# Audio-WestlakeU/FN-SSL

Measured on AMD Instinct MI355X. Metric: TF-frames/sec DP-IPD forward, 4-mic 257-bin x 300-frame, higher is better.
Workload: dtype f32; 1 GPU; BASELINE configs[1]: FN-SSL (online) DP-IPD forward, waveform->STFT->features->3x(full-band BiLSTM + narrow-band LSTM)->head; 32 utterances/GPU x 4 mics ('MM' = 6 pairs) x 257 bins x 300 frames, fp32; frame = one STFT frame of one utterance; stream_chunk_frames=0, utterances_per_gpu=32, global_batch=32, mics=4, pairs_per_utterance=6, frames=300, bins=257, parallelism=dp1 (utterance shards, no collective), chunk_pairs=0

## Files before the change

### fn-ssl_amd/csrc/lstm_f32c.h

```cpp
#pragma once

#include "lstm_static.h"

namespace fnssl_lstm {

constexpr int kF32cWaves = 16;

struct F32ClusterParams {
  unsigned* tags;
  unsigned* status;
  int clusters_per_dir;
  int groups_per_cluster;
  unsigned spin_limit;
  int stall_member;
  int rotate;
  int prio_mode;
};

template <int HH, int NV0, int NS0, int MODE, bool ABLRT = false, int DRIFT = 2, int NW_ = kF32cWaves, int GS = 1>
__global__ void __launch_bounds__(NW_ * 64) lstm_f32c_kernel(const LstmParams p, const F32ClusterParams cp) {
  constexpr int H = HH, NS = H / 16, NW = NW_;
  constexpr int NWS = NW / GS;
  static_assert((GS == 1 || GS == 4) && NW % GS == 0 && (NWS & (NWS - 1)) == 0, "gate split: whole slots, a power of two of them");
  constexpr bool SUM = (MODE & kSum) != 0, SAVE = (MODE & kSave) != 0;
  constexpr bool CAT = (MODE & kHas2) != 0;
  constexpr int QPS = 1 + NV0 + NS0 + NS;
  constexpr int XD = NW_ > 12 ? 4 : 8;
  constexpr bool STRH = H == 256 && GS == 1 && NW_ > 8;
  static_assert((CAT ? NS0 == 1 : !(NV0 && NS0)) && (NV0 == 0 || NV0 % XD == 0) && (H == 128 || H == 256),
                "blocks of src0, or its remainder alone, or blocks of src0 + the remainder quad of src2");
  static_assert(H == 128 || NW_ <= 8 || STRH, "H = 256 with the row of h_{t-1} held: at most two waves per SIMD (register budget)");
  static_assert(!STRH || (NV0 >= XD && (NV0 + NS) % XD == 0), "streamed row: the ring depth divides the block count");
  static_assert(GS == 1 || (!SAVE && !ABLRT), "gate split: inference kernels only");
  extern __shared__ __attribute__((aligned(16))) char smem[];
  const int ABL = ABLRT ? p.ablate : 0;

  const int b = blockIdx.x;
  const int m = (b >> 3) % NS;
  const int cl = ((b >> 3) / NS) * 8 + (b & 7);
  if (cl >= cp.clusters_per_dir * p.ndir) return;
  const int dir = cl / cp.clusters_per_dir;
  const int ck = cl - dir * cp.clusters_per_dir;
  const int g0 = ck * cp.groups_per_cluster;
  const int g1 = g0 + cp.groups_per_cluster < p.ntasks ? g0 + cp.groups_per_cluster : p.ntasks;
  if (__hip_atomic_load(cp.status, __ATOMIC_RELAXED, __HIP_MEMORY_SCOPE_AGENT) != 0) return;
  if (cl == 0 && m == cp.stall_member) return;

  const int lane = threadIdx.x & 63;
  const int n = lane & 15, g = lane >> 4;
  const int w = __builtin_amdgcn_readfirstlane((int)(threadIdx.x >> 6));
  const int ws = GS == 1 ? w : (w >> 2);
  const int gate = GS == 1 ? 0 : (w & 3);
  const bool rev = dir == 1;
  const unsigned vlane = lane * 16;

  {
    const v4f* src = reinterpret_cast<const v4f*>(reinterpret_cast<const char*>(p.wpack[dir]) + (size_t)(m * QPS) * 4096);
    v4f* dst = reinterpret_cast<v4f*>(smem);
    for (int i = threadIdx.x; i < QPS * 4 * 64; i += NW * 64) dst[i] = src[i];
  }
  char* const xch = smem + QPS * 4096;
  unsigned* const xcnt = reinterpret_cast<unsigned*>(xch + NWS * 2 * 4 * 1024);
  if (GS > 1 && threadIdx.x < NWS) xcnt[threadIdx.x] = 0;
  __syncthreads();
  const char* const lds_rd = smem + lane * 16;
  auto rec = [&](int q, int j) { return *reinterpret_cast<const v4f*>(lds_rd + (q * 4 + j) * 1024); };
  auto rec1 = [&](int q, int j) { return *reinterpret_cast<const float*>(lds_rd + (q * 4 + j) * 1024 + 4 * gate); };

  const unsigned st0 = (unsigned)(p.src0.st * 4), sto = (unsigned)(p.out_st * 4), stk = SUM ? (unsigned)(p.skip.st * 4) : 0u;
  const unsigned st2 = CAT ? (unsigned)(p.src2.st * 4) : 0u;
  const unsigned cy = (unsigned)p.carry;
  unsigned* const tag_cl = cp.tags + (size_t)cl * cp.groups_per_cluster * NS;
  const v4f zero4 = v4f{0.f, 0.f, 0.f, 0.f};

  unsigned pub_val = 0;
  unsigned* pub_tag = nullptr;
  auto pub_flush = [&]() {
    if (pub_tag) {
      asm volatile("s_waitcnt vmcnt(0)" ::: "memory");
      if (lane == 0) __hip_atomic_store(pub_tag, pub_val, __ATOMIC_RELAXED, __HIP_MEMORY_SCOPE_AGENT);
      pub_tag = nullptr;
    }
  };

  struct Grp {
    unsigned vo0, voo, vok, voo2, vo2 = 0;
    bool valid;
    int task, step;
  };
  auto locate = [&](int task, int qo0, int qi0, Grp& gr, rsrc_t& rx0, rsrc_t& ro, rsrc_t& rsk, rsrc_t& ro2, rsrc_t& rx2) {
    const int q0 = task * 16;
    gr.valid = q0 + n < p.nseq;
    const int d = q0 + n < p.nseq ? n : p.nseq - 1 - q0;
    const bool crossed = qi0 + d >= p.q_inner;
    auto one = [&](const float* base, long long so, long long si, int extra, unsigned& voff) {
      const long long delta = (long long)d * si + (crossed ? so - (long long)p.q_inner * si : 0ll);
      voff = (unsigned)(delta * 4) + (unsigned)(extra * 4);
      return make_rsrc(base + ((long long)qo0 * so + (long long)qi0 * si));
    };
    rx0 = one(p.src0.p, p.src0.so, p.src0.si, (NS0 && !CAT) ? g : 4 * g, gr.vo0);
    if constexpr (CAT) rx2 = one(p.src2.p, p.src2.so, p.src2.si, g, gr.vo2);
    ro = one(p.out, p.out_so, p.out_si, dir * H + 4 * g, gr.voo);
    gr.vok = gr.voo2 = 0;
    rsk = SUM ? one(p.skip.p, p.skip.so, p.skip.si, dir * H + 4 * g, gr.vok) : rx0;
    ro2 = SUM ? one(p.out_sum, p.out_so, p.out_si, dir * H + 4 * g, gr.voo2) : ro;
  };
  auto tt_of = [&](int step) { return (unsigned)(rev ? p.nsteps - 1 - step : step); };
  auto rc_of = [&](int task) {
    return make_rsrc(cell_record<NS>(p.cscratch, p.ntasks, dir, task));
  };

  if (g0 + ws >= g1) return;
  unsigned long long clk0 = 0, rt0 = 0;
  if (ABLRT && (ABL & 512)) {
    clk0 = __builtin_amdgcn_s_memtime();
    rt0 = __builtin_amdgcn_s_memrealtime();
  }
  bool dead = false;
  auto bounded_wait = [&](auto ready, auto reload, int sleep, unsigned code) {
    for (unsigned spins = 0; !ready(); ++spins) {
      if (GS > 1) __builtin_amdgcn_s_sleep(1); else if (sleep == 8) __builtin_amdgcn_s_sleep(8); else __builtin_amdgcn_s_sleep(16);
      reload();
      const bool out = spins > cp.spin_limit;
      if (out || (spins & 63) == 63) {
        if (out) {
          if (lane == 0) __hip_atomic_store(cp.status, code | (unsigned)(cl & 0xffff), __ATOMIC_RELAXED, __HIP_MEMORY_SCOPE_AGENT);
          return false;
        }
        if (__hip_atomic_load(cp.status, __ATOMIC_RELAXED, __HIP_MEMORY_SCOPE_AGENT) != 0) return false;
      }
    }
    return true;
  };
  const int NGR = g1 - g0;
  const bool rot = cp.rotate && NGR >= 2 * NWS;
  const int FULL = rot ? (NGR / NWS) * NWS : NGR, LEFT = NGR - FULL;
  const bool single = GS == 1 && g0 + ws + NWS >= g1;
  Grp cur, nxt;
  rsrc_t rx0, ro, rsk, ro2, rx2, nrx0, nro, nrsk, nro2, nrx2;
  v4f xr[XD];
  float xs0 = 0.f;
  v4f cprev = zero4, skipv = zero4;
  unsigned tagv = 0, tagd = 0;
  auto request = [&](const Grp& gr, rsrc_t qx0, rsrc_t qsk, bool with_c, bool with_x = true) {
    const unsigned tt = tt_of(gr.step);
    if (!(ABL & 8)) {
      if constexpr (NV0 > 0) if (with_x) static_for<XD>([&](auto v) { xr[v.value] = bld4(qx0, gr.vo0, tt * st0 + 64 * v.value); });
      if constexpr (NS0 > 0 && !CAT) xs0 = bld1(qx0, gr.vo0, tt * st0);
    }
    if (SUM && !(ABL & 64)) skipv = bld4(qsk, gr.vok, tt * stk + 64 * m);
    if (gr.step > 0 || cy) {
      if (gr.step > 0 && !(ABL & 256))
        tagv = __hip_atomic_load(tag_cl + (size_t)(gr.task - g0) * NS + (lane & (NS - 1)), __ATOMIC_RELAXED, __HIP_MEMORY_SCOPE_AGENT);
      if (GS == 1 && with_c && !(ABL & 64)) cprev = bld4_l2(rc_of(gr.task), vlane, m * 1024);
    }
    if (DRIFT > 0 && !(ABL & 256) && gr.task - DRIFT * NWS >= g0)
      tagd = __hip_atomic_load(tag_cl + (size_t)(gr.task - DRIFT * NWS - g0) * NS + (lane & (NS - 1)), __ATOMIC_RELAXED, __HIP_MEMORY_SCOPE_AGENT);
  };
  cur.task = g0 + ws;
  cur.step = 0;
  unsigned iter = 0;
  const int qo_first = (cur.task * 16) / p.q_inner, qi_first = cur.task * 16 - qo_first * p.q_inner;
  int qo0 = qo_first, qi0 = qi_first;
  locate(cur.task, qo0, qi0, cur, rx0, ro, rsk, ro2, rx2);
  request(cur, rx0, rsk, true);
  if constexpr (CAT) xs0 = bld1(rx2, cur.vo2, tt_of(0) * st2);

  for (;;) {
    const int step = cur.step, task = cur.task;
    const unsigned tt = tt_of(step);
    const unsigned o0 = tt * st0, oo = (tt + cy) * sto;
    const unsigned op = (rev ? tt + 1 : tt - 1 + cy) * sto;
    const rsrc_t rc = rc_of(task);
    unsigned* const tag_g = tag_cl + (size_t)(task - g0) * NS;
    if (single && (step > 0 || cy) && !(ABL & 64)) cprev = bld4_l2(rc, vlane, m * 1024);
    const bool late_c = GS > 1 || task >= g0 + FULL;
    v4f cprev_cur = (step > 0 || cy) ? cprev : zero4;
    const v4f skip_cur = skipv;

    v4f hold[STRH ? 1 : NS];
    auto fetch_h = [&]() {
      if (DRIFT > 0 && !(ABL & 4) && !dead && task - DRIFT * NWS >= g0) {
        unsigned* const tag_d = tag_cl + (size_t)(task - DRIFT * NWS - g0) * NS;
        dead = !bounded_wait([&]() { return __builtin_amdgcn_ballot_w64(tagd < (unsigned)step + 1) == 0; },
                             [&]() { tagd = __hip_atomic_load(tag_d + (lane & (NS - 1)), __ATOMIC_RELAXED, __HIP_MEMORY_SCOPE_AGENT); }, 8, 0x40000u);
      }
      if ((step > 0 || cy) && !(ABL & 16)) {
        if (step > 0 && !(ABL & 4) && !dead)
          dead = !bounded_wait([&]() { return __builtin_amdgcn_ballot_w64(tagv < (unsigned)step) == 0; },
                               [&]() { tagv = __hip_atomic_load(tag_g + (lane & (NS - 1)), __ATOMIC_RELAXED, __HIP_MEMORY_SCOPE_AGENT); }, 16, 0x30000u);
        if (late_c && !(ABL & 64)) cprev_cur = bld4_l2(rc, vlane, m * 1024);
        if constexpr (!STRH) {
#pragma unroll
          for (int s = 0; s < NS; ++s) hold[s] = bld4_l2(ro, cur.voo, op + 64 * s);
        }
      } else if constexpr (!STRH) {
#pragma unroll
        for (int s = 0; s < NS; ++s) hold[s] = (ABL & 16) ? cprev : zero4;
      }
    };
    const bool hrow = step > 0 || cy;
    auto hblock = [&](int j) { return hrow ? bld4_l2(ro, cur.voo, op + 64 * j) : zero4; };

    if (cp.prio_mode == 2) __builtin_amdgcn_s_setprio(2);
    v4f acc[4];
    v4f ra[4];
    v4f acc1 = zero4;
    float rb[4] = {0.f, 0.f, 0.f, 0.f};
    if constexpr (GS == 1) {
      acc[0] = rec(0, 0);
      acc[1] = rec(0, 1);
      acc[2] = rec(0, 2);
      acc[3] = rec(0, 3);
      static_for<4>([&](auto j) { ra[j.value] = rec(1, j.value); });
    } else {
      acc1 = rec(0, gate);
      static_for<4>([&](auto j) { rb[j.value] = rec1(1, j.value); });
    }
    auto quad = [&](auto qc, float b0, float b1, float b2, float b3) {
      constexpr int Q = decltype(qc)::value;
      if constexpr (GS > 1) {
        acc1 = __builtin_amdgcn_mfma_f32_16x16x4f32(rb[0], b0, acc1, 0, 0, 0);
        if constexpr (Q + 1 < QPS) rb[0] = rec1(Q + 1, 0);
        acc1 = __builtin_amdgcn_mfma_f32_16x16x4f32(rb[1], b1, acc1, 0, 0, 0);
        if constexpr (Q + 1 < QPS) rb[1] = rec1(Q + 1, 1);
        acc1 = __builtin_amdgcn_mfma_f32_16x16x4f32(rb[2], b2, acc1, 0, 0, 0);
        if constexpr (Q + 1 < QPS) rb[2] = rec1(Q + 1, 2);
        acc1 = __builtin_amdgcn_mfma_f32_16x16x4f32(rb[3], b3, acc1, 0, 0, 0);
        if constexpr (Q + 1 < QPS) rb[3] = rec1(Q + 1, 3);
        return;
      }
      MFMA4(acc, ra[0], b0);
      __builtin_amdgcn_sched_barrier(0);
      if constexpr (Q + 1 < QPS) if (!(ABL & 128)) ra[0] = rec(Q + 1, 0);
      __builtin_amdgcn_sched_barrier(0);
      MFMA4(acc, ra[1], b1);
      __builtin_amdgcn_sched_barrier(0);
      if constexpr (Q + 1 < QPS) if (!(ABL & 128)) ra[1] = rec(Q + 1, 1);
      __builtin_amdgcn_sched_barrier(0);
      MFMA4(acc, ra[2], b2);
      __builtin_amdgcn_sched_barrier(0);
      if constexpr (Q + 1 < QPS) if (!(ABL & 128)) ra[2] = rec(Q + 1, 2);
      __builtin_amdgcn_sched_barrier(0);
      MFMA4(acc, ra[3], b3);
      __builtin_amdgcn_sched_barrier(0);
      if constexpr (Q + 1 < QPS) if (!(ABL & 128)) ra[3] = rec(Q + 1, 3);
      __builtin_amdgcn_sched_barrier(0);
    };
    auto quad1 = [&](auto qc, float b0) {
      constexpr int Q = decltype(qc)::value;
      if constexpr (GS > 1) {
        acc1 = __builtin_amdgcn_mfma_f32_16x16x4f32(rb[0], b0, acc1, 0, 0, 0);
        if constexpr (Q + 1 < QPS) static_for<4>([&](auto j) { rb[j.value] = rec1(Q + 1, j.value); });
        return;
      }
      MFMA4(acc, ra[0], b0);
      if constexpr (Q + 1 < QPS) static_for<4>([&](auto j) { ra[j.value] = rec(Q + 1, j.value); });
    };
    if constexpr (NV0 > 0) {
      static_for<NV0>([&](auto v) {
        constexpr int V = decltype(v)::value;
        if constexpr (STRH) {
          if constexpr (V == NV0 / 2) pub_flush();
          if constexpr (V == NV0 - XD) fetch_h();
        } else if constexpr (V == NV0 / 2) {
          pub_flush();
          fetch_h();
        }
        const v4f xb = xr[V % XD];
        quad(ic<1 + V>{}, xb.x, xb.y, xb.z, xb.w);
        if constexpr (V + XD < NV0) {
          if (!(ABL & 8)) xr[V % XD] = bld4(rx0, cur.vo0, o0 + 64 * (V + XD));
        } else if constexpr (STRH) {
          xr[V % XD] = hblock(V + XD - NV0);
        }
      });
      if constexpr (NS0 > 0) quad1(ic<1 + NV0>{}, xs0);
    } else {
      pub_flush();
      fetch_h();
      quad1(ic<1>{}, xs0);
    }
    bool seq_next = false;
    if (task < g0 + FULL && task + NWS < g0 + FULL) {
      nxt.task = task + NWS;
      nxt.step = step;
      seq_next = true;
    } else {
      const int j = (ws - step) & (NWS - 1);
      if (task < g0 + FULL && j < LEFT) {
        nxt.task = g0 + FULL + j;
        nxt.step = step;
      } else {
        nxt.task = g0 + ws;
        nxt.step = step + 1;
      }
    }
    const bool more = nxt.step < p.nsteps;
    if (more) {
      if (ABL & 1) {
        nxt.vo0 = cur.vo0; nxt.voo = cur.voo; nxt.vok = cur.vok; nxt.voo2 = cur.voo2; nxt.valid = cur.valid;
        nrx0 = rx0; nro = ro; nrsk = rsk; nro2 = ro2;
        if constexpr (CAT) {
          nxt.vo2 = cur.vo2;
          nrx2 = rx2;
        }
      } else {
        if (seq_next) {
          qi0 += 16 * NWS;
          while (qi0 >= p.q_inner) {
            qi0 -= p.q_inner;
            ++qo0;
          }
        } else if (nxt.step == step) {
          qo0 = (nxt.task * 16) / p.q_inner;
          qi0 = nxt.task * 16 - qo0 * p.q_inner;
        } else {
          qo0 = qo_first;
          qi0 = qi_first;
        }
        locate(nxt.task, qo0, qi0, nxt, nrx0, nro, nrsk, nro2, nrx2);
      }
      request(nxt, nrx0, nrsk, !single && nxt.task < g0 + FULL, !STRH);
      if constexpr (CAT) xs0 = bld1(nrx2, nxt.vo2, tt_of(nxt.step) * st2);
    }
    static_for<NS>([&](auto sp) {
      constexpr int SP = decltype(sp)::value;
      if constexpr (STRH) {
        constexpr int B = NV0 + SP, B2 = B + XD;
        const v4f hb = xr[B % XD];
        quad(ic<1 + NV0 + NS0 + SP>{}, hb.x, hb.y, hb.z, hb.w);
        if constexpr (B2 < NV0 + NS) {
          xr[B % XD] = hblock(B2 - NV0);
        } else {
          if (more) xr[B % XD] = bld4(nrx0, nxt.vo0, tt_of(nxt.step) * st0 + 64 * (B2 - NV0 - NS));
        }
      } else {
        quad(ic<1 + NV0 + NS0 + SP>{}, hold[SP].x, hold[SP].y, hold[SP].z, hold[SP].w);
      }
    });

    if (cp.prio_mode == 2) __builtin_amdgcn_s_setprio(0);
    if (dead) break;
    v4f cn, hn;
    if (ABL & 2) {
      cn = acc[1] + cprev_cur + acc[0];
      hn = acc[3] + acc[2];
    } else {
      v4f ig, fg, gg, og;
      if constexpr (GS == 1) {
        ig = sigmoid4(acc[0]);
        fg = sigmoid4(acc[1]);
        gg = tanh4(acc[2]);
        og = sigmoid4(acc[3]);
      } else {
        const v4f act = gate == 2 ? tanh4(acc1) : sigmoid4(acc1);
        v4f* const xb = reinterpret_cast<v4f*>(xch + (size_t)((ws * 2 + (int)(iter & 1u)) * 4) * 1024);
        xb[gate * 64 + lane] = act;
        asm volatile("s_waitcnt lgkmcnt(0)" ::: "memory");
        if (lane == 0) __hip_atomic_fetch_add(xcnt + ws, 1u, __ATOMIC_RELAXED, __HIP_MEMORY_SCOPE_WORKGROUP);
        const unsigned want = 4u * (iter + 1u);
        for (unsigned spins = 0;; ++spins) {
          if (__hip_atomic_load(xcnt + ws, __ATOMIC_RELAXED, __HIP_MEMORY_SCOPE_WORKGROUP) >= want) break;
          if (dead || ((spins & 63u) == 63u && __hip_atomic_load(cp.status, __ATOMIC_RELAXED, __HIP_MEMORY_SCOPE_AGENT) != 0u) ||
              spins > cp.spin_limit) {
            dead = true;
            break;
          }
          __builtin_amdgcn_s_sleep(1);
        }
        asm volatile("" ::: "memory");
        ig = xb[lane];
        fg = xb[64 + lane];
        gg = xb[128 + lane];
        og = xb[192 + lane];
        ++iter;
      }
      cn = cell4(fg, cprev_cur, ig, gg);
      hn = mul_rn4(og, tanh4(cn));
      if constexpr (SAVE) {
        const rsrc_t rres = make_rsrc(reinterpret_cast<const char*>(p.reserve) +
                                      ((size_t)dir * p.ntasks + task) * p.nsteps * (size_t)(NS * kReserveRecs * 1024));
        const unsigned rb = (tt * NS + m) * (kReserveRecs * 1024);
        bst4(ig, rres, vlane, rb);
        bst4(fg, rres, vlane, rb + 1024);
        bst4(gg, rres, vlane, rb + 2048);
        bst4(og, rres, vlane, rb + 3072);
        bst4(cn, rres, vlane, rb + 4096);
      }
    }
    asm("" : "+v"(hn.x), "+v"(hn.y), "+v"(hn.z), "+v"(hn.w));
    if (ABL & 32) asm volatile("" ::"v"(cn), "v"(hn));
    const bool storer = GS == 1 || gate == 0;
    if (storer && !(ABL & 32)) bst4(cn, rc, vlane, m * 1024);
    if (storer && cur.valid && !(ABL & 32)) {
      __builtin_amdgcn_raw_buffer_store_b128(__builtin_bit_cast(v4u, hn), ro, cur.voo, oo + 64 * m, 16);
      if (SUM) bst4(add_rn4(hn, skip_cur), ro2, cur.voo2, oo + 64 * m);
    }
    pub_val = __builtin_amdgcn_readfirstlane((unsigned)step + 1);
    pub_tag = ((ABL & 256) || !storer) ? nullptr : tag_g + m;
    if (GS > 1 || single) pub_flush();
    if (!more || dead) break;
    cur = nxt;
    rx0 = nrx0;
    ro = nro;
    rsk = nrsk;
    ro2 = nro2;
    if constexpr (CAT) rx2 = nrx2;
  }
  pub_flush();
  asm volatile("s_waitcnt vmcnt(0)" ::: "memory");
  if (ABLRT && (ABL & 512) && (w == 0 || w == 15) && lane == 0) {
    const unsigned long long c1 = __builtin_amdgcn_s_memtime(), r1 = __builtin_amdgcn_s_memrealtime();
    printf("f32c blk %d wave %d start %llu end %llu cycles %llu MHz %.1f\n", b, w, rt0, r1, c1 - clk0,
           (double)(c1 - clk0) / (double)(r1 - rt0) * 100.0);
  }
}

template <int HH, int NV0, int NS0, int MODE, bool ABLRT = false, int DRIFT = 2, int NW_ = kF32cWaves, int GS = 1>
int launch_f32c_k(const LstmParams& p, const F32ClusterParams& cp, hipStream_t st) {
  constexpr int NS = HH / 16;
  constexpr int QPS = 1 + NV0 + NS0 + NS;
  const size_t lds = (size_t)QPS * 4096 + (GS > 1 ? (size_t)(NW_ / GS) * 8192 + 64 : 0);
  static_assert(QPS * 4096 + (GS > 1 ? (NW_ / GS) * 8192 + 64 : 0) <= 160 * 1024, "LDS");
  auto k = lstm_f32c_kernel<HH, NV0, NS0, MODE, ABLRT, DRIFT, NW_, GS>;
  if (lds > 48 * 1024)
    FNSSL_HIP(hipFuncSetAttribute(reinterpret_cast<const void*>(k), hipFuncAttributeMaxDynamicSharedMemorySize, (int)lds));
  const int ncl = cp.clusters_per_dir * p.ndir;
  const int nwg = 8 * NS * ((ncl + 7) / 8);
  if (!cluster_grid_fits(reinterpret_cast<const void*>(k), NW_ * 64, lds, nwg)) return kNoCluster;
  if (p.dry) return FNSSL_OK;
  hipLaunchKernelGGL(k, dim3(nwg), dim3(NW_ * 64), lds, st, p, cp);
  FNSSL_CHECK_LAUNCH("lstm_f32c_kernel");
  return FNSSL_OK;
}

}
```

### fn-ssl_amd/csrc/lstm_f32c.hip

```cpp
#include <cstdlib>

#include "lstm_f32c.h"
#include "tuning.h"

namespace fnssl_lstm {

constexpr int kF32cWavesH256 = 16;
constexpr int kF32cWavesH256Split = 8;

static bool f32c_uniform(const LstmParams& p, int mode) {
  auto even = [&](long long so, long long si) { return si >= 0 && so == (long long)p.q_inner * si; };
  return even(p.src0.so, p.src0.si) && even(p.out_so, p.out_si) && (!(mode & kSum) || even(p.skip.so, p.skip.si)) &&
         (!(mode & kHas2) || even(p.src2.so, p.src2.si));
}

bool f32c_handles(const LstmParams& p, int H, int mode) {
  if (fnssl::tune(FNSSL_TUNE_NO_F32_CLUSTER)) return false;
  if ((H != 128 && H != 256) || p.ablate) return false;
  if (H == 128) {
    if (p.c2 != 0 || p.carry) return false;
    if (p.reserve && mode != 0) return false;
    if (!(p.c0 == 256 && (mode == kSum || mode == 0)) && !(p.c0 == 4 && mode == 0 && !fnssl::tune(FNSSL_TUNE_NO_F32C_B1))) return false;
  } else {
    if (p.ndir != 1 || p.c0 != 256 || fnssl::tune(FNSSL_TUNE_NO_F32_SMALL)) return false;
    const bool plain = p.c2 == 0 && (mode == 0 || mode == kSum), cat = p.c2 == 4 && (mode == kHas2 || mode == (kHas2 | kSum));
    if (!plain && !cat) return false;
    if (p.reserve && ((mode & kSum) || p.carry)) return false;
  }
  auto grows = [&](long long so, long long si) { return si >= 0 && so >= (long long)(p.q_inner - 1) * si; };
  if (!f32c_uniform(p, mode) &&
      (p.q_inner < 16 || !grows(p.src0.so, p.src0.si) || !grows(p.out_so, p.out_si) ||
       ((mode & kSum) && !grows(p.skip.so, p.skip.si)) || ((mode & kHas2) && !grows(p.src2.so, p.src2.si))))
    return false;
  const int ncu = cluster_cus();
  if (ncu < (H / 16) * p.ndir) return false;
  const long long groups = (long long)p.ntasks * p.ndir;
  if (const int mg = fnssl::tune(FNSSL_TUNE_F32C_MIN_GROUPS, 1, 1 << 30)) {
    if (groups < mg) return false;
  }
  if (p.reserve) {
    if (fnssl::tune(FNSSL_TUNE_TRAIN_NO_F32_CLUSTER)) return false;
    return true;
  }
  if (H == 256) {
    const long long full = 12LL * ncu, rounds = (groups + full - 1) / full;
    return groups < full || groups * 100 < rounds * full * 97;
  }
  return !fnssl::tune(FNSSL_TUNE_NO_F32_SMALL) || groups >= 12LL * ncu;
}

int forward_f32c(LstmParams p, int H, int mode, size_t cluster_bytes, hipStream_t st) {
  if (f32c_uniform(p, mode)) p.q_inner = p.nseq;
  const int ncu = cluster_cus();
  const int members = H / 16;
  F32ClusterParams cp;
  cp.clusters_per_dir = (ncu / members) / p.ndir;
  cp.groups_per_cluster = (p.ntasks + cp.clusters_per_dir - 1) / cp.clusters_per_dir;
  cp.status = reinterpret_cast<unsigned*>(p.cluster_ws);
  cp.tags = reinterpret_cast<unsigned*>(p.cluster_ws + 256);
  cp.spin_limit = cluster_spin_limit();
  cp.stall_member = cluster_test_stall();
  cp.rotate = !fnssl::tune(FNSSL_TUNE_F32C_NO_ROTATE);
  cp.prio_mode = fnssl::tune(FNSSL_TUNE_F32C_PRIO, 9, 9) ? 0 : 2;
  const size_t tag_bytes = (size_t)p.ndir * cp.clusters_per_dir * cp.groups_per_cluster * members * sizeof(unsigned);
  FNSSL_REQUIRE(256 + tag_bytes <= cluster_bytes, "lstm_forward: the cluster kernel's tags exceed the workspace's cluster area");
  if (!p.dry) FNSSL_HIP(hipMemsetAsync(p.cluster_ws, 0, 256 + tag_bytes, st));
  const int gs_knob = fnssl::tune(FNSSL_TUNE_F32C_GATE_SPLIT, 1, 4);
  const bool gsplit = gs_knob ? gs_knob == 4 : cp.groups_per_cluster <= 1;
  if (H == 256) {
    constexpr int W = kF32cWavesH256;
    if (p.reserve)
      return p.c2 == 4 ? launch_f32c_k<256, 16, 1, kHas2 | kSave, false, 2, W>(p, cp, st) : launch_f32c_k<256, 16, 0, kSave, false, 2, W>(p, cp, st);
    if (gsplit) {
      if (mode == (kHas2 | kSum)) return launch_f32c_k<256, 16, 1, kHas2 | kSum, false, 2, kF32cWavesH256Split, 4>(p, cp, st);
      if (mode == kHas2) return launch_f32c_k<256, 16, 1, kHas2, false, 2, kF32cWavesH256Split, 4>(p, cp, st);
      if (mode == kSum) return launch_f32c_k<256, 16, 0, kSum, false, 2, kF32cWavesH256Split, 4>(p, cp, st);
      return launch_f32c_k<256, 16, 0, 0, false, 2, kF32cWavesH256Split, 4>(p, cp, st);
    }
    if (cp.groups_per_cluster <= kF32cWavesH256Split) {
      constexpr int W8 = kF32cWavesH256Split;
      if (mode == (kHas2 | kSum)) return launch_f32c_k<256, 16, 1, kHas2 | kSum, false, 2, W8>(p, cp, st);
      if (mode == kHas2) return launch_f32c_k<256, 16, 1, kHas2, false, 2, W8>(p, cp, st);
      if (mode == kSum) return launch_f32c_k<256, 16, 0, kSum, false, 2, W8>(p, cp, st);
      return launch_f32c_k<256, 16, 0, 0, false, 2, W8>(p, cp, st);
    }
    if (mode == (kHas2 | kSum)) return launch_f32c_k<256, 16, 1, kHas2 | kSum, false, 2, W>(p, cp, st);
    if (mode == kHas2) return launch_f32c_k<256, 16, 1, kHas2, false, 2, W>(p, cp, st);
    if (mode == kSum) return launch_f32c_k<256, 16, 0, kSum, false, 2, W>(p, cp, st);
    return launch_f32c_k<256, 16, 0, 0, false, 2, W>(p, cp, st);
  }
  if (gsplit && !p.reserve) {
    if (p.c0 == 4) return launch_f32c_k<128, 0, 1, 0, false, 2, kF32cWaves, 4>(p, cp, st);
    if (mode == kSum) return launch_f32c_k<128, 16, 0, kSum, false, 2, kF32cWaves, 4>(p, cp, st);
    return launch_f32c_k<128, 16, 0, 0, false, 2, kF32cWaves, 4>(p, cp, st);
  }
#ifdef FNSSL_BUILD_ABLATE
  if (const int abl = env_int("FNSSL_F32C_ABL", 1, 1023)) {
    p.ablate = abl;
    if (mode == kSum) return launch_f32c_k<128, 16, 0, kSum, true>(p, cp, st);
    if (p.c0 == 4) return launch_f32c_k<128, 0, 1, 0, true>(p, cp, st);
  }
  p.ablate = 0;
#endif
  if (p.reserve) return p.c0 == 4 ? launch_f32c_k<128, 0, 1, kSave>(p, cp, st) : launch_f32c_k<128, 16, 0, kSave>(p, cp, st);
  if (p.c0 == 4) return launch_f32c_k<128, 0, 1, 0>(p, cp, st);
  if (mode == kSum) return launch_f32c_k<128, 16, 0, kSum>(p, cp, st);
  return launch_f32c_k<128, 16, 0, 0>(p, cp, st);
}

}
```

### fn-ssl_amd/csrc/runtime.hip

```cpp
#include <atomic>
#include <cstring>
#include <map>
#include <mutex>
#include <string>
#include <vector>

#include "common.h"
#include "tuning.h"

namespace fnssl {

int device_cus() {
  static std::mutex mu;
  static int cache[64] = {0};
  int dev = 0;
  if (hipGetDevice(&dev) != hipSuccess || dev < 0 || dev >= 64) return 256;
  std::lock_guard<std::mutex> lk(mu);
  if (cache[dev] == 0) {
    int n = 0;
    if (hipDeviceGetAttribute(&n, hipDeviceAttributeMultiprocessorCount, dev) != hipSuccess || n <= 0) n = 256;
    cache[dev] = n;
  }
  return cache[dev];
}


static thread_local char g_err[512] = "";

namespace {
std::mutex g_tuning_mu;
fnssl_tuning g_default_tuning = {sizeof(fnssl_tuning), {0}};
std::atomic<unsigned> g_tuning_version{1};
thread_local fnssl_tuning g_thread_tuning = {sizeof(fnssl_tuning), {0}};
thread_local unsigned g_thread_version = 0;
thread_local const fnssl_tuning* g_call_tuning = nullptr;
const char* const kTuneNames[] = {
    "LSTM_NO_STATIC",
    "NO_STATIC3",
    "NO_STATIC2",
    "NO_STATIC_IPDNET",
    "LSTM_SPLIT",
    "SPLIT4_MAX_H256",
    "LSTM_VARIANT_H128",
    "LSTM_VARIANT_H256",
    "LSTM_CHQ",
    "NO_F32_CLUSTER",
    "NO_F32C_B1",
    "TRAIN_NO_F32_CLUSTER",
    "F32C_NO_ROTATE",
    "F32C_PRIO",
    "NO_CLUSTER",
    "NO_CLUSTER_B1",
    "NO_CLUSTER_H128",
    "CLUSTER_SPREAD",
    "BF16P_DRAIN",
    "BF16W_SOLO",
    "BWD_NO_CLUSTER",
    "BWD_CLUSTER_MIN_GROUPS",
    "BWD_CLUSTER_NO_ROTATE",
    "BWDC_NO_PREFETCH",
    "BWDC_NO_TOKEN",
    "BWDC_WAVES16",
    "FWD_RING",
    "BWD_RING",
    "TRAIN_SPLIT",
    "TRAIN_NO_STATIC",
    "NO_FWD2",
    "NO_BWD2",
    "SN_SCALAR",
    "STFT_PER_FRAME",
    "CLUSTER_SPIN_LIMIT",
    "CLUSTER_TEST_STALL",
    "RESERVED_CUS",
    "NO_F32_SMALL",
    "F32C_MIN_GROUPS",
    "F32C_GATE_SPLIT",
    "CLUSTER_FULL_TILES",
    "NO_STATIC4"};
constexpr int kTuneNamed = (int)(sizeof(kTuneNames) / sizeof(kTuneNames[0]));
static_assert(kTuneNamed <= FNSSL_TUNE_COUNT, "more knob names than slots");
static_assert(kTuneNamed == FNSSL_TUNE_NO_STATIC4 + 1, "knob names out of step with include/fnssl.h");
}

const fnssl_tuning& tuning() {
  if (g_call_tuning) return *g_call_tuning;
  const unsigned v = g_tuning_version.load(std::memory_order_acquire);
  if (v != g_thread_version) {
    std::lock_guard<std::mutex> lk(g_tuning_mu);
    g_thread_tuning = g_default_tuning;
    g_thread_version = g_tuning_version.load(std::memory_order_relaxed);
  }
  return g_thread_tuning;
}

TuningScope::TuningScope(const fnssl_tuning* t) : prev_(g_call_tuning), active_(false) {
  if (t && t->struct_bytes == sizeof(fnssl_tuning)) {
    g_call_tuning = t;
    active_ = true;
  }
}
TuningScope::~TuningScope() {
  if (active_) g_call_tuning = prev_;
}

void set_error(const char* fmt, ...) {
  va_list ap;
  va_start(ap, fmt);
  vsnprintf(g_err, sizeof(g_err), fmt, ap);
  va_end(ap);
}

namespace {
struct Rec {
  const char* name;
  double flops;
  hipEvent_t e0, e1;
};
std::mutex g_mu;
std::vector<Rec> g_recs;
bool g_timing = false;
char g_select[64] = "";
}

TimedLaunch::TimedLaunch(const char* name, hipStream_t s, double flops)
    : name_(name), s_(s), flops_(flops) {
  if (!g_timing || !name) return;
  if (g_select[0] && std::strcmp(g_select, name) != 0) return;
  if (hipEventCreate(&e0_) != hipSuccess) {
    e0_ = nullptr;
    return;
  }
  (void)hipEventRecord(e0_, s_);
}

TimedLaunch::~TimedLaunch() {
  if (!e0_) return;
  hipEvent_t e1 = nullptr;
  if (hipEventCreate(&e1) != hipSuccess) {
    (void)hipEventDestroy(e0_);
    return;
  }
  (void)hipEventRecord(e1, s_);
  std::lock_guard<std::mutex> lk(g_mu);
  g_recs.push_back(Rec{name_, flops_, e0_, e1});
}

}

extern "C" int fnssl_tuning_set(const fnssl_tuning* t) {
  FNSSL_REQUIRE(!t || t->struct_bytes == sizeof(fnssl_tuning), "tuning_set: struct_bytes %u, this library's fnssl_tuning has %zu",
                t ? t->struct_bytes : 0u, sizeof(fnssl_tuning));
  std::lock_guard<std::mutex> lk(fnssl::g_tuning_mu);
  fnssl::g_default_tuning = t ? *t : fnssl_tuning{sizeof(fnssl_tuning), {0}};
  fnssl::g_tuning_version.fetch_add(1, std::memory_order_release);
  return FNSSL_OK;
}

extern "C" int fnssl_tuning_get(fnssl_tuning* t) {
  FNSSL_REQUIRE(t != nullptr, "tuning_get: NULL");
  std::lock_guard<std::mutex> lk(fnssl::g_tuning_mu);
  *t = fnssl::g_default_tuning;
  return FNSSL_OK;
}

// ... 141 lines not shown
```

### include/fnssl.h

```cpp
#ifndef FNSSL_H_
#define FNSSL_H_

#include <stddef.h>

#ifdef __cplusplus
extern "C" {
#endif

#define FNSSL_ABI_VERSION 19

#define FNSSL_OK 0
#define FNSSL_E_INVALID (-1)
#define FNSSL_E_HIP (-2)
#define FNSSL_E_WORKSPACE (-3)

#define FNSSL_CH_MODE_M 0
#define FNSSL_CH_MODE_MM 1

#define FNSSL_WIN_LEN 512
#define FNSSL_HOP 256
#define FNSSL_NBIN 257
#define FNSSL_NF 256
#define FNSSL_SEG_FRAMES 12

int fnssl_abi_version(void);
const char* fnssl_last_error(void);


#define FNSSL_TUNE_LSTM_NO_STATIC 0
#define FNSSL_TUNE_NO_STATIC3 1
#define FNSSL_TUNE_NO_STATIC2 2
#define FNSSL_TUNE_NO_STATIC_IPDNET 3
#define FNSSL_TUNE_LSTM_SPLIT 4
#define FNSSL_TUNE_SPLIT4_MAX_H256 5
#define FNSSL_TUNE_LSTM_VARIANT_H128 6
#define FNSSL_TUNE_LSTM_VARIANT_H256 7
#define FNSSL_TUNE_LSTM_CHQ 8
#define FNSSL_TUNE_NO_F32_CLUSTER 9
#define FNSSL_TUNE_NO_F32C_B1 10
#define FNSSL_TUNE_TRAIN_NO_F32_CLUSTER 11
#define FNSSL_TUNE_F32C_NO_ROTATE 12
#define FNSSL_TUNE_F32C_PRIO 13
#define FNSSL_TUNE_NO_CLUSTER 14
#define FNSSL_TUNE_NO_CLUSTER_B1 15
#define FNSSL_TUNE_NO_CLUSTER_H128 16
#define FNSSL_TUNE_CLUSTER_SPREAD 17
#define FNSSL_TUNE_BF16P_DRAIN 18
#define FNSSL_TUNE_BF16W_SOLO 19
#define FNSSL_TUNE_BWD_NO_CLUSTER 20
#define FNSSL_TUNE_BWD_CLUSTER_MIN_GROUPS 21
#define FNSSL_TUNE_BWD_CLUSTER_NO_ROTATE 22
#define FNSSL_TUNE_BWDC_NO_PREFETCH 23
#define FNSSL_TUNE_BWDC_NO_TOKEN 24
#define FNSSL_TUNE_BWDC_WAVES16 25
#define FNSSL_TUNE_FWD_RING 26
#define FNSSL_TUNE_BWD_RING 27
#define FNSSL_TUNE_TRAIN_SPLIT 28
#define FNSSL_TUNE_TRAIN_NO_STATIC 29
#define FNSSL_TUNE_NO_FWD2 30
#define FNSSL_TUNE_NO_BWD2 31
#define FNSSL_TUNE_SN_SCALAR 32
#define FNSSL_TUNE_STFT_PER_FRAME 33
#define FNSSL_TUNE_CLUSTER_SPIN_LIMIT 34
#define FNSSL_TUNE_CLUSTER_TEST_STALL 35
#define FNSSL_TUNE_RESERVED_CUS 36
#define FNSSL_TUNE_NO_F32_SMALL 37
#define FNSSL_TUNE_F32C_MIN_GROUPS 38
#define FNSSL_TUNE_F32C_GATE_SPLIT 39
#define FNSSL_TUNE_CLUSTER_FULL_TILES 40
#define FNSSL_TUNE_NO_STATIC4 41
#define FNSSL_TUNE_COUNT 48

typedef struct fnssl_tuning {
  unsigned struct_bytes;
  int knob[FNSSL_TUNE_COUNT];
} fnssl_tuning;

int fnssl_tuning_set(const fnssl_tuning* t);
int fnssl_tuning_get(fnssl_tuning* t);
const char* fnssl_tuning_name(int index);

int fnssl_occupy_cus(int nblocks, int lds_bytes, unsigned* stop, int max_ms, void* stream);


int fnssl_num_frames(int ns);

int fnssl_num_pairs(int nch, int ch_mode);

int fnssl_stft(const float* sig, int nb, int ns, int nch,
               long long sb, long long sn, long long sc,
               float* spec, float* magsum, void* stream);

int fnssl_num_frames_ex(int ns, int hop, int center);
int fnssl_stft_ex(const float* sig, int nb, int ns, int nch,
                  long long sb, long long sn, long long sc, int hop, int center,
                  float* spec, float* magsum, void* stream);

int fnssl_forgetting_coefs(int nt, int sample_length, float* a, float* b);

int fnssl_pair_features(const float* spec, const float* magsum,
                        const float* coef_a, const float* coef_b,
                        int nb, int nch, int nt, int ch_mode, float eps,
                        float* mu, float* x, int layout, void* stream);

int fnssl_nchw_to_seq(const float* x, int n, int c, int nf, int nt, float* y, void* stream);


typedef struct {
  const float* p;
  long long so, si, st;
} fnssl_view;

typedef struct {
  fnssl_view src0, src1, src2;
  int c0, c2;
  float* out;
  long long out_so, out_si, out_st;
  fnssl_view skip;
  float* out_sum;
  int hidden;
  int ndir;
  int nseq;
  int q_inner;
  int nsteps;
  const float* wpack[2];
  float* workspace;
  size_t workspace_bytes;
  int variant;
  float* reserve;
  size_t reserve_bytes;
  int carry_state;
  int precision;
  int f32_mask;
  unsigned* fallback_count;
  const fnssl_tuning* tuning;
} fnssl_lstm_desc;

#define FNSSL_PRECISION_FP32 0
#define FNSSL_PRECISION_BF16 1
#define FNSSL_PRECISION_BF16W 2

size_t fnssl_lstm_packed_floats_bf16w(int c0, int c2, int hidden);
int fnssl_lstm_pack_bf16w(const float* w_ih, const float* w_hh, const float* b_ih, const float* b_hh,
                          int c0, int c2, int hidden, float* packed);

size_t fnssl_lstm_packed_floats_bf16(int c0, int c2, int hidden);
int fnssl_lstm_pack_bf16(const float* w_ih, const float* w_hh, const float* b_ih, const float* b_hh,
                         int c0, int c2, int hidden, float* packed);

size_t fnssl_lstm_packed_floats(int c0, int c2, int hidden);

int fnssl_lstm_pack(const float* w_ih, const float* w_hh, const float* b_ih, const float* b_hh,
                    int c0, int c2, int hidden, float* packed);
// ... 340 lines not shown
```

Baseline: 17360 frames/s.

## Cut f32c LSTM register pressure: shared residual layout, late cell/skip loads, pointer groups

Result: no change. 17460 frames/s, median of 6 (+0.6%).

```diff
diff --git a/fn-ssl_amd/csrc/lstm_f32c.h b/fn-ssl_amd/csrc/lstm_f32c.h
--- a/fn-ssl_amd/csrc/lstm_f32c.h
+++ b/fn-ssl_amd/csrc/lstm_f32c.h
@@ -17,7 +17,7 @@
   int prio_mode;
 };
 
-template <int HH, int NV0, int NS0, int MODE, bool ABLRT = false, int DRIFT = 2, int NW_ = kF32cWaves, int GS = 1>
+template <int HH, int NV0, int NS0, int MODE, bool ABLRT = false, int DRIFT = 2, int NW_ = kF32cWaves, int GS = 1, bool SHR = false>
 __global__ void __launch_bounds__(NW_ * 64) lstm_f32c_kernel(const LstmParams p, const F32ClusterParams cp) {
   constexpr int H = HH, NS = H / 16, NW = NW_;
   constexpr int NWS = NW / GS;
@@ -32,6 +32,8 @@
   static_assert(H == 128 || NW_ <= 8 || STRH, "H = 256 with the row of h_{t-1} held: at most two waves per SIMD (register budget)");
   static_assert(!STRH || (NV0 >= XD && (NV0 + NS) % XD == 0), "streamed row: the ring depth divides the block count");
   static_assert(GS == 1 || (!SAVE && !ABLRT), "gate split: inference kernels only");
+  constexpr bool LATE = !STRH && NV0 > 0;
+  static_assert(!SHR || (SUM && NV0 > 0), "shared-layout residual: a fused residual beside 16-channel input blocks");
   extern __shared__ __attribute__((aligned(16))) char smem[];
   const int ABL = ABLRT ? p.ablate : 0;
 
@@ -63,11 +65,20 @@
   unsigned* const xcnt = reinterpret_cast<unsigned*>(xch + NWS * 2 * 4 * 1024);
   if (GS > 1 && threadIdx.x < NWS) xcnt[threadIdx.x] = 0;
   __syncthreads();
+  unsigned seg1 = 1u << 16, seg2 = 2u << 16;
+  asm("" : "+v"(seg1));
+  asm("" : "+v"(seg2));
   const char* const lds_rd = smem + lane * 16;
-  auto rec = [&](int q, int j) { return *reinterpret_cast<const v4f*>(lds_rd + (q * 4 + j) * 1024); };
-  auto rec1 = [&](int q, int j) { return *reinterpret_cast<const float*>(lds_rd + (q * 4 + j) * 1024 + 4 * gate); };
-
-  const unsigned st0 = (unsigned)(p.src0.st * 4), sto = (unsigned)(p.out_st * 4), stk = SUM ? (unsigned)(p.skip.st * 4) : 0u;
+  const char* const lds_seg[3] = {lds_rd, lds_rd + seg1, lds_rd + seg2};
+  auto rec_at = [&](int off) { return lds_seg[off >> 16] + (off & 0xffff); };
+  auto rec = [&](int q, int j) { return *reinterpret_cast<const v4f*>(rec_at((q * 4 + j) * 1024)); };
+  auto rec1 = [&](int q, int j) { return *reinterpret_cast<const float*>(rec_at((q * 4 + j) * 1024) + 4 * gate); };
+
+  const unsigned st0 = (unsigned)(p.src0.st * 4), sto = (unsigned)(p.out_st * 4);
+  const unsigned stk = SHR ? st0 : SUM ? (unsigned)(p.skip.st * 4) : 0u;
+  const long long dsk = SHR ? reinterpret_cast<const char*>(p.skip.p) - reinterpret_cast<const char*>(p.src0.p) : 0ll;
+  const long long dsum = SHR ? reinterpret_cast<const char*>(p.out_sum) - reinterpret_cast<const char*>(p.out) : 0ll;
+  const unsigned cok = SHR ? (unsigned)(dir * H * 4) : 0u;
   const unsigned st2 = CAT ? (unsigned)(p.src2.st * 4) : 0u;
   const unsigned cy = (unsigned)p.carry;
   unsigned* const tag_cl = cp.tags + (size_t)cl * cp.groups_per_cluster * NS;
@@ -84,27 +95,34 @@
   };
 
   struct Grp {
-    unsigned vo0, voo, vok, voo2, vo2 = 0;
+    unsigned vo0, voo, vok = 0, voo2 = 0, vo2 = 0;
     bool valid;
     int task, step;
-  };
-  auto locate = [&](int task, int qo0, int qi0, Grp& gr, rsrc_t& rx0, rsrc_t& ro, rsrc_t& rsk, rsrc_t& ro2, rsrc_t& rx2) {
+    const char *bx0, *bo, *bsk = nullptr, *bo2 = nullptr, *bx2 = nullptr;
+    __device__ __forceinline__ rsrc_t rx0() const { return make_rsrc(bx0); }
+    __device__ __forceinline__ rsrc_t ro() const { return make_rsrc(bo); }
+    __device__ __forceinline__ rsrc_t rx2() const { return make_rsrc(bx2); }
+  };
+  auto locate = [&](int task, int qo0, int qi0, Grp& gr) {
     const int q0 = task * 16;
     gr.valid = q0 + n < p.nseq;
     const int d = q0 + n < p.nseq ? n : p.nseq - 1 - q0;
     const bool crossed = qi0 + d >= p.q_inner;
     auto one = [&](const float* base, long long so, long long si, int extra, unsigned& voff) {
-      const long long delta = (long long)d * si + (crossed ? so - (long long)p.q_inner * si : 0ll);
-      voff = (unsigned)(delta * 4) + (unsigned)(extra * 4);
-      return make_rsrc(base + ((long long)qo0 * so + (long long)qi0 * si));
+      const unsigned sob = (unsigned)so * 4u, sib = (unsigned)si * 4u;
+      voff = (unsigned)d * sib + (crossed ? sob - (unsigned)p.q_inner * sib : 0u) + (unsigned)(extra * 4);
+      return reinterpret_cast<const char*>(base) + ((unsigned long long)(unsigned)qo0 * sob + (unsigned long long)(unsigned)qi0 * sib);
     };
-    rx0 = one(p.src0.p, p.src0.so, p.src0.si, (NS0 && !CAT) ? g : 4 * g, gr.vo0);
-    if constexpr (CAT) rx2 = one(p.src2.p, p.src2.so, p.src2.si, g, gr.vo2);
-    ro = one(p.out, p.out_so, p.out_si, dir * H + 4 * g, gr.voo);
-    gr.vok = gr.voo2 = 0;
-    rsk = SUM ? one(p.skip.p, p.skip.so, p.skip.si, dir * H + 4 * g, gr.vok) : rx0;
-    ro2 = SUM ? one(p.out_sum, p.out_so, p.out_si, dir * H + 4 * g, gr.voo2) : ro;
-  };
+    gr.bx0 = one(p.src0.p, p.src0.so, p.src0.si, (NS0 && !CAT) ? g : 4 * g, gr.vo0);
+    if constexpr (CAT) gr.bx2 = one(p.src2.p, p.src2.so, p.src2.si, g, gr.vo2);
+    gr.bo = one(p.out, p.out_so, p.out_si, dir * H + 4 * g, gr.voo);
+    if constexpr (SUM && !SHR) {
+      gr.bsk = one(p.skip.p, p.skip.so, p.skip.si, dir * H + 4 * g, gr.vok);
+      gr.bo2 = one(p.out_sum, p.out_so, p.out_si, dir * H + 4 * g, gr.voo2);
+    }
+  };
+  auto rsk_of = [&](const Grp& gr) { return make_rsrc(SHR ? gr.bx0 + dsk : gr.bsk); };
+  auto ro2_of = [&](const Grp& gr) { return make_rsrc(SHR ? gr.bo + dsum : gr.bo2); };
   auto tt_of = [&](int step) { return (unsigned)(rev ? p.nsteps - 1 - step : step); };
   auto rc_of = [&](int task) {
     return make_rsrc(cell_record<NS>(p.cscratch, p.ntasks, dir, task));
@@ -136,47 +154,48 @@
   const bool rot = cp.rotate && NGR >= 2 * NWS;
   const int FULL = rot ? (NGR / NWS) * NWS : NGR, LEFT = NGR - FULL;
   const bool single = GS == 1 && g0 + ws + NWS >= g1;
-  Grp cur, nxt;
-  rsrc_t rx0, ro, rsk, ro2, rx2, nrx0, nro, nrsk, nro2, nrx2;
+  Grp ga, gb;
   v4f xr[XD];
   float xs0 = 0.f;
   v4f cprev = zero4, skipv = zero4;
   unsigned tagv = 0, tagd = 0;
-  auto request = [&](const Grp& gr, rsrc_t qx0, rsrc_t qsk, bool with_c, bool with_x = true) {
+  auto request = [&](const Grp& gr, bool with_c, bool with_x = true) {
     const unsigned tt = tt_of(gr.step);
+    const rsrc_t qx0 = gr.rx0();
     if (!(ABL & 8)) {
       if constexpr (NV0 > 0) if (with_x) static_for<XD>([&](auto v) { xr[v.value] = bld4(qx0, gr.vo0, tt * st0 + 64 * v.value); });
       if constexpr (NS0 > 0 && !CAT) xs0 = bld1(qx0, gr.vo0, tt * st0);
     }
-    if (SUM && !(ABL & 64)) skipv = bld4(qsk, gr.vok, tt * stk + 64 * m);
+    if (SUM && !LATE && !(ABL & 64)) skipv = bld4(rsk_of(gr), SHR ? gr.vo0 : gr.vok, tt * stk + 64 * m + cok);
     if (gr.step > 0 || cy) {
       if (gr.step > 0 && !(ABL & 256))
         tagv = __hip_atomic_load(tag_cl + (size_t)(gr.task - g0) * NS + (lane & (NS - 1)), __ATOMIC_RELAXED, __HIP_MEMORY_SCOPE_AGENT);
-      if (GS == 1 && with_c && !(ABL & 64)) cprev = bld4_l2(rc_of(gr.task), vlane, m * 1024);
+      if (GS == 1 && !LATE && with_c && !(ABL & 64)) cprev = bld4_l2(rc_of(gr.task), vlane, m * 1024);
     }
     if (DRIFT > 0 && !(ABL & 256) && gr.task - DRIFT * NWS >= g0)
       tagd = __hip_atomic_load(tag_cl + (size_t)(gr.task - DRIFT * NWS - g0) * NS + (lane & (NS - 1)), __ATOMIC_RELAXED, __HIP_MEMORY_SCOPE_AGENT);
   };
-  cur.task = g0 + ws;
-  cur.step = 0;
+  ga.task = g0 + ws;
+  ga.step = 0;
   unsigned iter = 0;
-  const int qo_first = (cur.task * 16) / p.q_inner, qi_first = cur.task * 16 - qo_first * p.q_inner;
+  const int qo_first = (ga.task * 16) / p.q_inner, qi_first = ga.task * 16 - qo_first * p.q_inner;
   int qo0 = qo_first, qi0 = qi_first;
-  locate(cur.task, qo0, qi0, cur, rx0, ro, rsk, ro2, rx2);
-  request(cur, rx0, rsk, true);
-  if constexpr (CAT) xs0 = bld1(rx2, cur.vo2, tt_of(0) * st2);
-
-  for (;;) {
+  locate(ga.task, qo0, qi0, ga);
+  request(ga, true);
+  if constexpr (CAT) xs0 = bld1(ga.rx2(), ga.vo2, tt_of(0) * st2);
+
+  auto group_step = [&](Grp& cur, Grp& nxt) __attribute__((always_inline)) -> bool {
     const int step = cur.step, task = cur.task;
+    const rsrc_t rx0 = cur.rx0(), ro = cur.ro();
     const unsigned tt = tt_of(step);
     const unsigned o0 = tt * st0, oo = (tt + cy) * sto;
     const unsigned op = (rev ? tt + 1 : tt - 1 + cy) * sto;
     const rsrc_t rc = rc_of(task);
     unsigned* const tag_g = tag_cl + (size_t)(task - g0) * NS;
-    if (single && (step > 0 || cy) && !(ABL & 64)) cprev = bld4_l2(rc, vlane, m * 1024);
-    const bool late_c = GS > 1 || task >= g0 + FULL;
-    v4f cprev_cur = (step > 0 || cy) ? cprev : zero4;
-    const v4f skip_cur = skipv;
+    if (single && !LATE && (step > 0 || cy) && !(ABL & 64)) cprev = bld4_l2(rc, vlane, m * 1024);
+    const bool late_c = LATE || GS > 1 || task >= g0 + FULL;
+    v4f cprev_cur = (LATE || step > 0 || cy) ? cprev : zero4;
+    v4f skip_cur = skipv;
 
     v4f hold[STRH ? 1 : NS];
     auto fetch_h = [&]() {
@@ -189,14 +208,24 @@
         if (step > 0 && !(ABL & 4) && !dead)
           dead = !bounded_wait([&]() { return __builtin_amdgcn_ballot_w64(tagv < (unsigned)step) == 0; },
                                [&]() { tagv = __hip_atomic_load(tag_g + (lane & (NS - 1)), __ATOMIC_RELAXED, __HIP_MEMORY_SCOPE_AGENT); }, 16, 0x30000u);
-        if (late_c && !(ABL & 64)) cprev_cur = bld4_l2(rc, vlane, m * 1024);
+        if (late_c && !LATE && !(ABL & 64)) cprev_cur = bld4_l2(rc, vlane, m * 1024);
         if constexpr (!STRH) {
 #pragma unroll
           for (int s = 0; s < NS; ++s) hold[s] = bld4_l2(ro, cur.voo, op + 64 * s);
         }
       } else if constexpr (!STRH) {
+        v4f z = (ABL & 16) ? cprev : zero4;
+        asm volatile("" : "+v"(z));
 #pragma unroll
-        for (int s = 0; s < NS; ++s) hold[s] = (ABL & 16) ? cprev : zero4;
+        for (int s = 0; s < NS; ++s) hold[s] = z;
+      }
+      if constexpr (LATE) {
+        if (step > 0 || cy) {
+          if (!(ABL & 64)) cprev_cur = bld4_l2(rc, vlane, m * 1024);
+        } else {
+          asm volatile("" : "+v"(cprev_cur));
+        }
+        if (SUM && !(ABL & 64)) skip_cur = bld4(rsk_of(cur), SHR ? cur.vo0 : cur.vok, tt * stk + 64 * m + cok);
       }
     };
     const bool hrow = step > 0 || cy;
@@ -299,12 +328,10 @@
     const bool more = nxt.step < p.nsteps;
     if (more) {
       if (ABL & 1) {
-        nxt.vo0 = cur.vo0; nxt.voo = cur.voo; nxt.vok = cur.vok; nxt.voo2 = cur.voo2; nxt.valid = cur.valid;
-        nrx0 = rx0; nro = ro; nrsk = rsk; nro2 = ro2;
-        if constexpr (CAT) {
-          nxt.vo2 = cur.vo2;
-          nrx2 = rx2;
-        }
+        const int nt = nxt.task, ns = nxt.step;
+        nxt = cur;
+        nxt.task = nt;
+        nxt.step = ns;
       } else {
         if (seq_next) {
           qi0 += 16 * NWS;
@@ -319,10 +346,10 @@
           qo0 = qo_first;
           qi0 = qi_first;
         }
-        locate(nxt.task, qo0, qi0, nxt, nrx0, nro, nrsk, nro2, nrx2);
-      }
-      request(nxt, nrx0, nrsk, !single && nxt.task < g0 + FULL, !STRH);
-      if constexpr (CAT) xs0 = bld1(nrx2, nxt.vo2, tt_of(nxt.step) * st2);
+        locate(nxt.task, qo0, qi0, nxt);
+      }
+      request(nxt, !single && nxt.task < g0 + FULL, !STRH);
+      if constexpr (CAT) xs0 = bld1(nxt.rx2(), nxt.vo2, tt_of(nxt.step) * st2);
     }
     static_for<NS>([&](auto sp) {
       constexpr int SP = decltype(sp)::value;
@@ -333,7 +360,7 @@
         if constexpr (B2 < NV0 + NS) {
           xr[B % XD] = hblock(B2 - NV0);
         } else {
-          if (more) xr[B % XD] = bld4(nrx0, nxt.vo0, tt_of(nxt.step) * st0 + 64 * (B2 - NV0 - NS));
+          if (more) xr[B % XD] = bld4(nxt.rx0(), nxt.vo0, tt_of(nxt.step) * st0 + 64 * (B2 - NV0 - NS));
         }
       } else {
         quad(ic<1 + NV0 + NS0 + SP>{}, hold[SP].x, hold[SP].y, hold[SP].z, hold[SP].w);
@@ -341,7 +368,7 @@
     });
 
     if (cp.prio_mode == 2) __builtin_amdgcn_s_setprio(0);
-    if (dead) break;
+    if (dead) return false;
     v4f cn, hn;
     if (ABL & 2) {
       cn = acc[1] + cprev_cur + acc[0];
@@ -395,19 +422,14 @@
     if (storer && !(ABL & 32)) bst4(cn, rc, vlane, m * 1024);
     if (storer && cur.valid && !(ABL & 32)) {
       __builtin_amdgcn_raw_buffer_store_b128(__builtin_bit_cast(v4u, hn), ro, cur.voo, oo + 64 * m, 16);
-      if (SUM) bst4(add_rn4(hn, skip_cur), ro2, cur.voo2, oo + 64 * m);
+      if (SUM) bst4(add_rn4(hn, skip_cur), ro2_of(cur), SHR ? cur.voo : cur.voo2, oo + 64 * m);
     }
     pub_val = __builtin_amdgcn_readfirstlane((unsigned)step + 1);
     pub_tag = ((ABL & 256) || !storer) ? nullptr : tag_g + m;
     if (GS > 1 || single) pub_flush();
-    if (!more || dead) break;
-    cur = nxt;
-    rx0 = nrx0;
-    ro = nro;
-    rsk = nrsk;
-    ro2 = nro2;
-    if constexpr (CAT) rx2 = nrx2;
-  }
+    return more && !dead;
+  };
+  while (group_step(ga, gb)) ga = gb;
   pub_flush();
   asm volatile("s_waitcnt vmcnt(0)" ::: "memory");
   if (ABLRT && (ABL & 512) && (w == 0 || w == 15) && lane == 0) {
@@ -417,13 +439,13 @@
   }
 }
 
-template <int HH, int NV0, int NS0, int MODE, bool ABLRT = false, int DRIFT = 2, int NW_ = kF32cWaves, int GS = 1>
+template <int HH, int NV0, int NS0, int MODE, bool ABLRT = false, int DRIFT = 2, int NW_ = kF32cWaves, int GS = 1, bool SHR = false>
 int launch_f32c_k(const LstmParams& p, const F32ClusterParams& cp, hipStream_t st) {
   constexpr int NS = HH / 16;
   constexpr int QPS = 1 + NV0 + NS0 + NS;
   const size_t lds = (size_t)QPS * 4096 + (GS > 1 ? (size_t)(NW_ / GS) * 8192 + 64 : 0);
   static_assert(QPS * 4096 + (GS > 1 ? (NW_ / GS) * 8192 + 64 : 0) <= 160 * 1024, "LDS");
-  auto k = lstm_f32c_kernel<HH, NV0, NS0, MODE, ABLRT, DRIFT, NW_, GS>;
+  auto k = lstm_f32c_kernel<HH, NV0, NS0, MODE, ABLRT, DRIFT, NW_, GS, SHR>;
   if (lds > 48 * 1024)
     FNSSL_HIP(hipFuncSetAttribute(reinterpret_cast<const void*>(k), hipFuncAttributeMaxDynamicSharedMemorySize, (int)lds));
   const int ncl = cp.clusters_per_dir * p.ndir;
diff --git a/fn-ssl_amd/csrc/lstm_f32c.hip b/fn-ssl_amd/csrc/lstm_f32c.hip
--- a/fn-ssl_amd/csrc/lstm_f32c.hip
+++ b/fn-ssl_amd/csrc/lstm_f32c.hip
@@ -12,6 +12,18 @@
   auto even = [&](long long so, long long si) { return si >= 0 && so == (long long)p.q_inner * si; };
   return even(p.src0.so, p.src0.si) && even(p.out_so, p.out_si) && (!(mode & kSum) || even(p.skip.so, p.skip.si)) &&
          (!(mode & kHas2) || even(p.src2.so, p.src2.si));
+}
+
+static bool f32c_shared_residual(const LstmParams& p, int mode) {
+  return (mode & kSum) && p.skip.so == p.src0.so && p.skip.si == p.src0.si && p.skip.st == p.src0.st &&
+         !fnssl::tune(FNSSL_TUNE_F32C_GENERAL_RESIDUAL);
+}
+
+template <int HH, int NV0, int NS0, int MODE, bool ABLRT = false, int NW_ = kF32cWaves, int GS = 1>
+static int launch_f32c_sum(bool shared, const LstmParams& p, const F32ClusterParams& cp, hipStream_t st) {
+  static_assert((MODE & kSum) != 0, "fused residual");
+  return shared ? launch_f32c_k<HH, NV0, NS0, MODE, ABLRT, 2, NW_, GS, true>(p, cp, st)
+                : launch_f32c_k<HH, NV0, NS0, MODE, ABLRT, 2, NW_, GS, false>(p, cp, st);
 }
 
 bool f32c_handles(const LstmParams& p, int H, int mode) {
@@ -67,44 +79,46 @@
   if (!p.dry) FNSSL_HIP(hipMemsetAsync(p.cluster_ws, 0, 256 + tag_bytes, st));
   const int gs_knob = fnssl::tune(FNSSL_TUNE_F32C_GATE_SPLIT, 1, 4);
   const bool gsplit = gs_knob ? gs_knob == 4 : cp.groups_per_cluster <= 1;
+  const bool shr = f32c_shared_residual(p, mode);
   if (H == 256) {
     constexpr int W = kF32cWavesH256;
     if (p.reserve)
       return p.c2 == 4 ? launch_f32c_k<256, 16, 1, kHas2 | kSave, false, 2, W>(p, cp, st) : launch_f32c_k<256, 16, 0, kSave, false, 2, W>(p, cp, st);
     if (gsplit) {
-      if (mode == (kHas2 | kSum)) return launch_f32c_k<256, 16, 1, kHas2 | kSum, false, 2, kF32cWavesH256Split, 4>(p, cp, st);
+      if (mode == (kHas2 | kSum)) return launch_f32c_sum<256, 16, 1, kHas2 | kSum, false, kF32cWavesH256Split, 4>(shr, p, cp, st);
       if (mode == kHas2) return launch_f32c_k<256, 16, 1, kHas2, false, 2, kF32cWavesH256Split, 4>(p, cp, st);
-      if (mode == kSum) return launch_f32c_k<256, 16, 0, kSum, false, 2, kF32cWavesH256Split, 4>(p, cp, st);
+      if (mode == kSum) return launch_f32c_sum<256, 16, 0, kSum, false, kF32cWavesH256Split, 4>(shr, p, cp, st);
       return launch_f32c_k<256, 16, 0, 0, false, 2, kF32cWavesH256Split, 4>(p, cp, st);
     }
     if (cp.groups_per_cluster <= kF32cWavesH256Split) {
       constexpr int W8 = kF32cWavesH256Split;
-      if (mode == (kHas2 | kSum)) return launch_f32c_k<256, 16, 1, kHas2 | kSum, false, 2, W8>(p, cp, st);
+      if (mode == (kHas2 | kSum)) return launch_f32c_sum<256, 16, 1, kHas2 | kSum, false, W8>(shr, p, cp, st);
       if (mode == kHas2) return launch_f32c_k<256, 16, 1, kHas2, false, 2, W8>(p, cp, st);
-      if (mode == kSum) return launch_f32c_k<256, 16, 0, kSum, false, 2, W8>(p, cp, st);
+      if (mode == kSum) return launch_f32c_sum<256, 16, 0, kSum, false, W8>(shr, p, cp, st);
       return launch_f32c_k<256, 16, 0, 0, false, 2, W8>(p, cp, st);
     }
-    if (mode == (kHas2 | kSum)) return launch_f32c_k<256, 16, 1, kHas2 | kSum, false, 2, W>(p, cp, st);
+    if (mode == (kHas2 | kSum)) return launch_f32c_sum<256, 16, 1, kHas2 | kSum, false, W>(shr, p, cp, st);
     if (mode == kHas2) return launch_f32c_k<256, 16, 1, kHas2, false, 2, W>(p, cp, st);
-    if (mode == kSum) return launch_f32c_k<256, 16, 0, kSum, false, 2, W>(p, cp, st);
+    if (mode == kSum) return launch_f32c_sum<256, 16, 0, kSum, false, W>(shr, p, cp, st);
     return launch_f32c_k<256, 16, 0, 0, false, 2, W>(p, cp, st);
   }
   if (gsplit && !p.reserve) {
     if (p.c0 == 4) return launch_f32c_k<128, 0, 1, 0, false, 2, kF32cWaves, 4>(p, cp, st);
-    if (mode == kSum) return launch_f32c_k<128, 16, 0, kSum, false, 2, kF32cWaves, 4>(p, cp, st);
+    if (mode == kSum) return launch_f32c_sum<128, 16, 0, kSum, false, kF32cWaves, 4>(shr, p, cp, st);
     return launch_f32c_k<128, 16, 0, 0, false, 2, kF32cWaves, 4>(p, cp, st);
   }
 #ifdef FNSSL_BUILD_ABLATE
   if (const int abl = env_int("FNSSL_F32C_ABL", 1, 1023)) {
     p.ablate = abl;
-    if (mode == kSum) return launch_f32c_k<128, 16, 0, kSum, true>(p, cp, st);
+    if (mode == kSum) return launch_f32c_sum<128, 16, 0, kSum, true>(shr, p, cp, st);
     if (p.c0 == 4) return launch_f32c_k<128, 0, 1, 0, true>(p, cp, st);
+    if (p.c0 == 256 && mode == 0) return launch_f32c_k<128, 16, 0, 0, true>(p, cp, st);
   }
   p.ablate = 0;
 #endif
   if (p.reserve) return p.c0 == 4 ? launch_f32c_k<128, 0, 1, kSave>(p, cp, st) : launch_f32c_k<128, 16, 0, kSave>(p, cp, st);
   if (p.c0 == 4) return launch_f32c_k<128, 0, 1, 0>(p, cp, st);
-  if (mode == kSum) return launch_f32c_k<128, 16, 0, kSum>(p, cp, st);
+  if (mode == kSum) return launch_f32c_sum<128, 16, 0, kSum>(shr, p, cp, st);
   return launch_f32c_k<128, 16, 0, 0>(p, cp, st);
 }
 
diff --git a/fn-ssl_amd/csrc/runtime.hip b/fn-ssl_amd/csrc/runtime.hip
--- a/fn-ssl_amd/csrc/runtime.hip
+++ b/fn-ssl_amd/csrc/runtime.hip
@@ -76,10 +76,11 @@
     "F32C_MIN_GROUPS",
     "F32C_GATE_SPLIT",
     "CLUSTER_FULL_TILES",
-    "NO_STATIC4"};
+    "NO_STATIC4",
+    "F32C_GENERAL_RESIDUAL"};
 constexpr int kTuneNamed = (int)(sizeof(kTuneNames) / sizeof(kTuneNames[0]));
 static_assert(kTuneNamed <= FNSSL_TUNE_COUNT, "more knob names than slots");
-static_assert(kTuneNamed == FNSSL_TUNE_NO_STATIC4 + 1, "knob names out of step with include/fnssl.h");
+static_assert(kTuneNamed == FNSSL_TUNE_F32C_GENERAL_RESIDUAL + 1, "knob names out of step with include/fnssl.h");
 }
 
 const fnssl_tuning& tuning() {
diff --git a/include/fnssl.h b/include/fnssl.h
--- a/include/fnssl.h
+++ b/include/fnssl.h
@@ -69,6 +69,7 @@
 #define FNSSL_TUNE_F32C_GATE_SPLIT 39
 #define FNSSL_TUNE_CLUSTER_FULL_TILES 40
 #define FNSSL_TUNE_NO_STATIC4 41
+#define FNSSL_TUNE_F32C_GENERAL_RESIDUAL 42
 #define FNSSL_TUNE_COUNT 48
 
 typedef struct fnssl_tuning {
```
